# SCZwangxiao/video-ReTaKe

Hardware: NVIDIA B200
Metric: 2048-frame DPSelect+PivotKV frames/s (higher is better)
Workload: dtype bf16

## Files before the change

### video-retake_b200/csrc/pivot_misc.cu

```cuda
#include <climits>

#include <stdlib.h>

#include "rtk_common.cuh"

namespace rtk {

struct RopeParams {
    int heads, L, D, n_pos, forward;
    long long stride_h, stride_l, out_stride_h, out_stride_l;
    int heads2;
    const __nv_bfloat16* x2;
    __nv_bfloat16* out2;
    long long stride_h2, stride_l2, out_stride_h2, out_stride_l2;
    int bound[6];
    float inv_scale2;
};

static bool mrope_bounds(int n_pos, const int32_t* sec, int64_t D, int bound[6]) {
    int acc = 0;
    for (int i = 0; i < 6; ++i) {
        acc += n_pos == 3 ? sec[i % 3] : 0;
        bound[i] = acc;
    }
    return n_pos != 3 || acc == D;
}

__device__ __forceinline__ int rope_pos_row(const RopeParams& p, int c) {
    if (p.n_pos == 1) return 0;
    int i = 0;
    while (i < 5 && c >= p.bound[i]) ++i;
    return i % 3;
}

__global__ void __launch_bounds__(256)
pivot_rope_table_kernel(const long long* __restrict__ pos, const float* __restrict__ inv_freq, RopeParams p, float scaling,
                        __nv_bfloat16* __restrict__ cos_t, __nv_bfloat16* __restrict__ sin_t) {
    pdl_enter();
    const int half = p.D >> 1;
    const long long total = (long long)p.L * p.D;
    for (long long i = (long long)blockIdx.x * blockDim.x + threadIdx.x; i < total; i += (long long)gridDim.x * blockDim.x) {
        const int c = (int)(i % p.D);
        const int l = (int)(i / p.D);
        const long long pv = pos[(size_t)rope_pos_row(p, c) * p.L + l];
        const float ang = inv_freq[c < half ? c : c - half] * (float)pv;
        cos_t[i] = __float2bfloat16_rn(cosf(ang) * scaling);
        sin_t[i] = __float2bfloat16_rn(sinf(ang) * scaling);
    }
}

__device__ __forceinline__ void rope_rotate_pair(float xa, float xb, float cosa, float sina, float cosb, float sinb, int forward,
                                                 float inv_scale2, __nv_bfloat16& oa, __nv_bfloat16& ob) {
    const float ta = round_bf16(xa * cosa), ra = round_bf16(-xb * sina);
    const float tb = round_bf16(xb * cosb), rb = round_bf16(xa * sinb);
    float ya, yb;
    if (forward) {
        ya = ta + ra;
        yb = tb + rb;
    } else {
        ya = round_bf16(ta - ra) * inv_scale2;
        yb = round_bf16(tb - rb) * inv_scale2;
    }
    oa = __float2bfloat16_rn(ya);
    ob = __float2bfloat16_rn(yb);
}

__device__ __forceinline__ void rope_table_entry(const RopeParams& p, const float* __restrict__ inv_freq, const long long* pv,
                                                 int c, float scaling, float& co, float& si) {
    const int half = p.D >> 1;
    const float ang = inv_freq[c < half ? c : c - half] * (float)pv[rope_pos_row(p, c)];
    co = __bfloat162float(__float2bfloat16_rn(cosf(ang) * scaling));
    si = __bfloat162float(__float2bfloat16_rn(sinf(ang) * scaling));
}

#ifndef RTK_UNROPE_TOK
#define RTK_UNROPE_TOK 2
#endif
constexpr int kUnropeTok = RTK_UNROPE_TOK;

__device__ __forceinline__ uint32_t sub_bf16x2_rn(uint32_t a, uint32_t b) {
    uint32_t d;
    asm("sub.rn.bf16x2 %0, %1, %2;" : "=r"(d) : "r"(a), "r"(b));
    return d;
// ... 154 lines not shown
#pragma unroll
            for (int e = 0; e < 8; ++e) {
                const int ca = c0 + e, cb = c0 + e + half;
                const size_t ia = ((size_t)rope_pos_row(p, ca) * p.L + l) * p.D + ca;
                const size_t ib = ((size_t)rope_pos_row(p, cb) * p.L + l) * p.D + cb;
                cav[e] = cos_t[ia]; sav[e] = sin_t[ia]; cbv[e] = cos_t[ib]; sbv[e] = sin_t[ib];
            }
        }
#pragma unroll
        for (int e = 0; e < 8; ++e)
            rope_rotate_pair(__bfloat162float(xl[e]), __bfloat162float(xh[e]), __bfloat162float(cav[e]), __bfloat162float(sav[e]),
                             __bfloat162float(cbv[e]), __bfloat162float(sbv[e]), p.forward, p.inv_scale2, ol[e], oh[e]);
        *reinterpret_cast<uint4*>(dst + c0) = ol4;
        *reinterpret_cast<uint4*>(dst + c0 + half) = oh4;
    }
}

bool key_elision_enabled();

struct KeyElide {
    const uint8_t* keymask[kMaxBatchLayers];
    int32_t* slot[kMaxBatchLayers];
    const __nv_bfloat16* k[kMaxBatchLayers];
    long long k_stride_h[kMaxBatchLayers], k_stride_l[kMaxBatchLayers];
    __nv_bfloat16* kc[kMaxBatchLayers];
    int32_t* n_keys;
    int L, KVH, D;
};

__global__ void __launch_bounds__(1024)
pivot_keymask_scan_kernel(const __grid_constant__ KeyElide e) {
    pdl_enter();
    __shared__ int wsum[32];
    const int layer = blockIdx.x, tid = threadIdx.x, lane = tid & 31, warp = tid >> 5;
    const uint8_t* __restrict__ m = e.keymask[layer];
    int32_t* __restrict__ slot = e.slot[layer];
    const int per = (e.L + 1023) / 1024;
    const int beg = min(tid * per, e.L), end = min(beg + per, e.L);
    int cnt = 0;
    for (int i = beg; i < end; ++i) cnt += !(m && m[i]);
    int inc = cnt;
#pragma unroll
    for (int o = 1; o < 32; o <<= 1) {
        const int n = __shfl_up_sync(0xffffffffu, inc, o);
        if (lane >= o) inc += n;
    }
    if (lane == 31) wsum[warp] = inc;
    __syncthreads();
    if (warp == 0) {
        const int w = wsum[lane];
        int winc = w;
#pragma unroll
        for (int o = 1; o < 32; o <<= 1) {
            const int n = __shfl_up_sync(0xffffffffu, winc, o);
            if (lane >= o) winc += n;
        }
        wsum[lane] = winc - w;
        if (lane == 31) e.n_keys[layer] = winc;
    }
    __syncthreads();
    int base = wsum[warp] + inc - cnt;
    for (int i = beg; i < end; ++i) slot[i] = (m && m[i]) ? -1 : base++;
}

__global__ void __launch_bounds__(256)
pivot_keys_compact_kernel(const __grid_constant__ KeyElide e) {
    pdl_enter();
    const int layer = blockIdx.y;
    const int vpr = e.D >> 3;
    const long long total = (long long)e.L * e.KVH * vpr;
    const int32_t* __restrict__ slot = e.slot[layer];
    for (long long i = (long long)blockIdx.x * blockDim.x + threadIdx.x; i < total; i += (long long)gridDim.x * blockDim.x) {
        const int v = (int)(i % vpr);
        const long long lh = i / vpr;
        const int h = (int)(lh % e.KVH);
        const int l = (int)(lh / e.KVH);
        const int sl = slot[l];
        if (sl < 0) continue;
        const uint4 w = __ldg(reinterpret_cast<const uint4*>(e.k[layer] + h * e.k_stride_h[layer] + l * e.k_stride_l[layer] + v * 8));
        *reinterpret_cast<uint4*>(e.kc[layer] + ((size_t)sl * e.KVH + h) * e.D + v * 8) = w;
    }
}

static int key_elide_prepare(KeyElide& ke, int n, ScoreBatch& sb, cudaStream_t st) {
    RTK_LAUNCH_PDL(pivot_keymask_scan_kernel, (unsigned)n, 1024, 0, st, ke);
    const long long total = (long long)ke.L * ke.KVH * (ke.D >> 3);
    long long gx = (total + 255) / 256;
    if (gx > 148 * 8) gx = 148 * 8;
    RTK_LAUNCH_PDL(pivot_keys_compact_kernel, dim3((unsigned)gx, (unsigned)n), 256, 0, st, ke);
    for (int i = 0; i < n; ++i) {
        sb.kc[i] = ke.kc[i];
        sb.slot[i] = ke.slot[i];
    }
    sb.n_keys = ke.n_keys;
    return 0;
}

static size_t key_elide_bytes(int64_t KVH, int64_t L, int64_t D) {
    return (((size_t)KVH * L * D * 2 + 255) & ~(size_t)255) + (((size_t)L * 4 + 255) & ~(size_t)255);
}

constexpr int kSelThreads = 1024;

__device__ void block_select_top(const uint32_t* keys, int L, int keep, int32_t* out_idx, int* sh ,
                                 int low_bit ) {
    const int tid = threadIdx.x, lane = tid & 31, warp = tid >> 5;
    const int per = (L + kSelThreads - 1) / kSelThreads;
    const int beg = min(tid * per, L), end = min(beg + per, L);
    uint32_t prefix = 0;
    for (int bit = 31; bit >= low_bit; --bit) {
        const uint32_t cand = prefix | (1u << bit);
        int cnt = 0;
        for (int i = beg; i < end; ++i) cnt += (keys[i] >= cand);
        cnt = __reduce_add_sync(0xffffffffu, cnt);
        int* buf = sh + 40 + 32 * (bit & 1);
        if (lane == 0) buf[warp] = cnt;
        __syncthreads();
        const int total = __reduce_add_sync(0xffffffffu, buf[lane]);
        if (total >= keep) prefix = cand;
    }
    __syncthreads();
    if (low_bit > 0 && (!(prefix & 0x80000000u) || (prefix >> low_bit) == (0xffffffffu >> low_bit)))
        prefix |= (1u << low_bit) - 1u;
    int gt = 0, eq = 0;
    for (int i = beg; i < end; ++i) { gt += (keys[i] > prefix); eq += (keys[i] == prefix); }
    auto block_excl_scan = [&](int v, int& total) {
        int inc = v;
#pragma unroll
        for (int o = 1; o < 32; o <<= 1) {
            const int n = __shfl_up_sync(0xffffffffu, inc, o);
            if (lane >= o) inc += n;
        }
        __syncthreads();
        if (lane == 31) sh[1 + warp] = inc;
        __syncthreads();
        if (warp == 0) {
            int w = sh[1 + lane], winc = w;
#pragma unroll
            for (int o = 1; o < 32; o <<= 1) {
                const int n = __shfl_up_sync(0xffffffffu, winc, o);
                if (lane >= o) winc += n;
            }
            sh[1 + lane] = winc - w;
            if (lane == 31) sh[33] = winc;
        }
        __syncthreads();
        total = sh[33];
        return sh[1 + warp] + inc - v;
    };
    int gt_total, eq_total;
    const int gt_before = block_excl_scan(gt, gt_total);
    const int eq_before = block_excl_scan(eq, eq_total);
    const int need = keep - gt_total;
    const int eq_taken_before = min(eq_before, need);
    int slot = gt_before + eq_taken_before;
    int eq_seen = eq_before;
    for (int i = beg; i < end; ++i) {
        const uint32_t k = keys[i];
        bool take = k > prefix;
        if (k == prefix) { take = eq_seen < need; ++eq_seen; }
        if (take) out_idx[slot++] = i;
    }
}

__device__ __forceinline__ void pivot_select_body(const __nv_bfloat16* __restrict__ head_scores, int KVH, int L,
                                                  const uint8_t* __restrict__ keymask, int keep, int32_t* __restrict__ keep_idx,
                                                  __nv_bfloat16* __restrict__ score_out, const long long* __restrict__ tpos,
                                                  long long* __restrict__ tmin_out) {
    extern __shared__ __align__(128) uint8_t smem[];
    uint32_t* keys = reinterpret_cast<uint32_t*>(smem);
    int* sh = reinterpret_cast<int*>(smem + (size_t)L * 4);
    const float rcp = 1.0f / (float)KVH;
// ... 388 lines not shown
    RTK_LAUNCH_PDL(pivot_rope_table_kernel, (unsigned)grid, 256, 0, (cudaStream_t)stream,  (const long long*)pos, inv_freq, p, attention_scaling, (__nv_bfloat16*)cos_out, (__nv_bfloat16*)sin_out);
    return 0;
}

static size_t align256(size_t x) { return (x + 255) & ~(size_t)255; }

extern "C" size_t rtk_pivot_update_batch_workspace_bytes(int64_t H, int64_t KVH, int64_t L, int64_t D, int64_t n_layers) {
    if (H < 1 || KVH < 1 || L < 1 || D < 1 || n_layers < 1) return 0;
    const size_t n = (size_t)(n_layers < kMaxBatchLayers ? n_layers : kMaxBatchLayers);
    return align256(rtk_pivot_score_workspace_bytes(H * (int64_t)n, L)) +
           n * (align256((size_t)H * L * D * 2) + align256((size_t)KVH * L * D * 2)) + align256(n * sizeof(long long)) + 256 +
           n * key_elide_bytes(KVH, L, D) + 256;
}

extern "C" size_t rtk_pivot_update_workspace_bytes(int64_t H, int64_t KVH, int64_t L, int64_t D) {
    return rtk_pivot_update_batch_workspace_bytes(H, KVH, L, D, 1);
}

#ifndef RTK_UNROT_TOKEN_MAJOR
#define RTK_UNROT_TOKEN_MAJOR 1
#endif

static int pivot_update_group(const rtk_pivot_update_args* a, int n, char* ws, cudaStream_t st) {
    const rtk_pivot_update_args& a0 = a[0];
    const int64_t H = a0.H, KVH = a0.KVH, L = a0.L, D = a0.D;
    const bool reforge = a0.reforge != 0;
    const int64_t uq_sh = RTK_UNROT_TOKEN_MAJOR ? D : L * D, uq_sl = RTK_UNROT_TOKEN_MAJOR ? H * D : D;
    const int64_t uk_sh = RTK_UNROT_TOKEN_MAJOR ? D : L * D, uk_sl = RTK_UNROT_TOKEN_MAJOR ? KVH * D : D;
    void* score_ws = ws;                ws += align256(rtk_pivot_score_workspace_bytes(H * n, L));
    char* qu0 = ws;                     ws += (size_t)n * align256((size_t)H * L * D * 2);
    char* ku0 = ws;                     ws += (size_t)n * align256((size_t)KVH * L * D * 2);
    long long* tmin = (long long*)ws;   ws += align256((size_t)n * sizeof(long long)) + 256;
    char* kc0 = ws;                     ws += (size_t)n * align256((size_t)KVH * L * D * 2);
    char* slot0 = ws;                   ws += (size_t)n * align256((size_t)L * 4);
    int32_t* nkeys_ws = (int32_t*)ws;

    BatchLayers t = {};
    ScoreBatch sb = {};
    sb.n = n; sb.H = H; sb.KVH = KVH; sb.L = L; sb.D = D;
    for (int i = 0; i < kMaxBatchLayers; ++i) {
        const rtk_pivot_update_args& x = a[i < n ? i : 0];
        char* qu = qu0 + (size_t)(i < n ? i : 0) * align256((size_t)H * L * D * 2);
        char* ku = ku0 + (size_t)(i < n ? i : 0) * align256((size_t)KVH * L * D * 2);
        t.q[i] = (const __nv_bfloat16*)x.q;       t.q_stride_h[i] = x.q_stride_h;     t.q_stride_l[i] = x.q_stride_l;
        t.k_in[i] = (const __nv_bfloat16*)x.k;    t.kin_stride_h[i] = x.k_stride_h;   t.kin_stride_l[i] = x.k_stride_l;
        t.qu[i] = (__nv_bfloat16*)qu;             t.ku[i] = (__nv_bfloat16*)ku;
        t.k[i] = reforge ? (const __nv_bfloat16*)ku : (const __nv_bfloat16*)x.k;
        t.k_stride_h[i] = reforge ? uk_sh : x.k_stride_h;
        t.k_stride_l[i] = reforge ? uk_sl : x.k_stride_l;
        t.v[i] = (const __nv_bfloat16*)x.v;       t.v_stride_h[i] = x.v_stride_h;     t.v_stride_l[i] = x.v_stride_l;
        t.pos[i] = (const long long*)x.pos;       t.keymask[i] = x.keymask;
        t.k_out[i] = (__nv_bfloat16*)x.k_out;     t.v_out[i] = (__nv_bfloat16*)x.v_out;
        t.out_stride_h[i] = x.out_stride_h;
        t.pos_out[i] = (long long*)x.pos_out;     t.pos_out_stride[i] = x.pos_out_stride > 0 ? x.pos_out_stride : x.keep;
        t.keep_idx[i] = x.keep_idx;               t.head_scores[i] = (const __nv_bfloat16*)x.head_scores;
        if (i < n) {
            sb.q[i] = reforge ? (const void*)qu : x.q;
            sb.k[i] = reforge ? (const void*)ku : x.k;
            sb.q_stride_h[i] = reforge ? uq_sh : x.q_stride_h;   sb.q_stride_l[i] = reforge ? uq_sl : x.q_stride_l;
            sb.k_stride_h[i] = reforge ? uk_sh : x.k_stride_h;   sb.k_stride_l[i] = reforge ? uk_sl : x.k_stride_l;
            sb.head_scores[i] = x.head_scores;
        }
    }
    RopeParams rp = {};
    rp.heads = (int)H; rp.L = (int)L; rp.D = (int)D; rp.n_pos = a0.n_pos; rp.forward = 0;
    rp.out_stride_h = uq_sh; rp.out_stride_l = uq_sl;
    rp.heads2 = (int)KVH; rp.out_stride_h2 = uk_sh; rp.out_stride_l2 = uk_sl;
    rp.inv_scale2 = a0.inv_scale2;
    mrope_bounds(a0.n_pos, a0.mrope_section, D, rp.bound);
    const bool xchg = a0.xchg_world > 1;
    const int64_t score_rows = a0.score_rows > 0 ? a0.score_rows : KVH;
    if (reforge && !a0.skip_score) {
        if (a0.inv_freq) {
            RTK_LAUNCH_PDL(pivot_unrope_qk_batch_kernel, dim3((unsigned)((L + kUnropeTok - 1) / kUnropeTok), (unsigned)n), 256, 0, st, t, a0.inv_freq,
                           a0.attention_scaling, rp);
        } else {
            rp.stride_h = a0.q_stride_h; rp.stride_l = a0.q_stride_l;
            rp.x2 = t.k_in[0]; rp.out2 = t.ku[0]; rp.stride_h2 = a0.k_stride_h; rp.stride_l2 = a0.k_stride_l;
            const int rc = rope_launch(a0.q, a0.cos, a0.sin, t.qu[0], rp, st);
            if (rc) return rc;
        }
    }
    if (!a0.skip_score) {
        bool any_mask = false;
        for (int i = 0; i < n; ++i) any_mask = any_mask || a[i].keymask != nullptr;
        if (any_mask && key_elision_enabled()) {
            KeyElide ke = {};
            ke.L = (int)L; ke.KVH = (int)KVH; ke.D = (int)D; ke.n_keys = nkeys_ws;
            for (int i = 0; i < kMaxBatchLayers; ++i) {
                const int j = i < n ? i : 0;
                ke.keymask[i] = a[j].keymask;
                ke.slot[i] = (int32_t*)(slot0 + (size_t)j * align256((size_t)L * 4));
                ke.k[i] = t.k[j]; ke.k_stride_h[i] = t.k_stride_h[j]; ke.k_stride_l[i] = t.k_stride_l[j];
                ke.kc[i] = (__nv_bfloat16*)(kc0 + (size_t)j * align256((size_t)KVH * L * D * 2));
            }
            int rc = key_elide_prepare(ke, n, sb, st);
            if (rc) return rc;
        }
        if (a0.ev_score_begin) cudaEventRecord((cudaEvent_t)a0.ev_score_begin, st);
        int rc = pivot_score_batch(sb, score_ws, rtk_pivot_score_workspace_bytes(H * n, L), st);
        if (rc) return rc;
        if (a0.ev_score_end) cudaEventRecord((cudaEvent_t)a0.ev_score_end, st);
    }
    if (a0.skip_select) {
        if (xchg) {
            XchgPutBatch xp = {};
            xp.n = (long long)KVH * L; xp.world = a0.xchg_world; xp.rank = a0.xchg_rank;
            for (int i = 0; i < n; ++i) {
                xp.src[i] = (const __nv_bfloat16*)a[i].head_scores;
                for (int r = 0; r < a0.xchg_world; ++r)
                    xp.dst[i][r] = (__nv_bfloat16*)a[i].xchg_scores[r] + (size_t)a0.xchg_rank * KVH * L;
            }
            RTK_LAUNCH_PDL(pivot_xchg_put_batch_kernel, (unsigned)n, 1024, 0, st, xp);
            XchgFlags xf = {};
            xf.world = a0.xchg_world; xf.rank = a0.xchg_rank; xf.epoch = a0.xchg_epoch;
            for (int r = 0; r < a0.xchg_world; ++r) xf.flags[r] = a0.xchg_flags[r];
            RTK_LAUNCH_PDL(pivot_xchg_flag_kernel, 1, 32, 0, st, xf);
        }
        return 0;
    }
    {
        const size_t smem = (size_t)L * 4 + 112 * 4;
        cudaError_t e = cudaFuncSetAttribute(pivot_select_batch_kernel, cudaFuncAttributeMaxDynamicSharedMemorySize, (int)smem);
        if (e != cudaSuccess) return (int)e;
        RTK_LAUNCH_PDL(pivot_select_batch_kernel, (unsigned)n, kSelThreads, smem, st, t, (int)score_rows, (int)L, (int)a0.keep,
                       reforge ? 1 : 0, tmin, (const uint32_t*)(xchg ? a0.xchg_flags[a0.xchg_rank] : nullptr),
                       xchg ? a0.xchg_world : 0, a0.xchg_epoch, xchg_timeout_ns());
    }
    {
        CompactParams p = {};
        p.KVH = (int)KVH; p.L = (int)L; p.D = (int)D; p.keep = (int)a0.keep; p.n_pos = a0.pos ? a0.n_pos : 0; p.reforge = a0.reforge;
        p.ratio = (float)((double)a0.keep / (double)L);
        RopeParams rq = {};
        rq.D = (int)D; rq.n_pos = a0.n_pos; rq.L = (int)a0.keep;
        for (int i = 0; i < 6; ++i) rq.bound[i] = rp.bound[i];
        RTK_LAUNCH_PDL(pivot_compact_rope_batch_kernel, dim3((unsigned)a0.keep, (unsigned)n), 128, 0, st, t, (const long long*)tmin,
                       a0.inv_freq, a0.attention_scaling, p, rq, (reforge && a0.inv_freq) ? 1 : 0);
    }
    return 0;
}

static int update_check(const rtk_pivot_update_args* layers, int64_t n, const void* workspace, size_t workspace_bytes) {
    if (!layers || n < 1 || !workspace) return RTK_E_BADARG;
    const rtk_pivot_update_args& a0 = layers[0];
    const bool scores = !a0.skip_score, selects = !a0.skip_select, xchg = a0.xchg_world > 1;
    if (!scores && !selects) return RTK_E_BADARG;
    if (a0.H < 1 || a0.KVH < 1 || a0.L < 1 || (selects && (a0.keep < 1 || a0.keep > a0.L))) return RTK_E_BADARG;
    if (a0.L > 16384 || a0.D % 16 != 0 || a0.D > 256) return RTK_E_UNSUPPORTED;
    if (scores && ((a0.D != 64 && a0.D != 128) || a0.H % a0.KVH != 0 || a0.H > 256)) return RTK_E_UNSUPPORTED;
    if (xchg) {
        if (n > kMaxBatchLayers) return RTK_E_UNSUPPORTED;
        if (a0.xchg_world > 8 || a0.xchg_rank < 0 || a0.xchg_rank >= a0.xchg_world || (scores && selects)) return RTK_E_BADARG;
    }
    if (a0.reforge && !a0.inv_freq && n > 1) return RTK_E_UNSUPPORTED;
    int bound[6];
    if (a0.reforge && (scores || a0.inv_freq) && !mrope_bounds(a0.n_pos, a0.mrope_section, a0.D, bound)) return RTK_E_UNSUPPORTED;
    if (((uintptr_t)workspace & 255u) != 0) return RTK_E_ALIGN;
    if (workspace_bytes < rtk_pivot_update_batch_workspace_bytes(a0.H, a0.KVH, a0.L, a0.D, n)) return RTK_E_WORKSPACE;
    for (int64_t i = 0; i < n; ++i) {
        const rtk_pivot_update_args& x = layers[i];
        if (!x.q || !x.k || !x.v || !x.k_out || !x.v_out || !x.keep_idx || !x.head_scores) return RTK_E_BADARG;
        if (x.H != a0.H || x.KVH != a0.KVH || x.L != a0.L || x.D != a0.D || x.keep != a0.keep || x.reforge != a0.reforge ||
            x.n_pos != a0.n_pos || x.inv_freq != a0.inv_freq || x.attention_scaling != a0.attention_scaling ||
            x.inv_scale2 != a0.inv_scale2 || x.skip_select != a0.skip_select || x.skip_score != a0.skip_score ||
            x.score_rows != a0.score_rows || x.xchg_world != a0.xchg_world || x.xchg_rank != a0.xchg_rank ||
            x.xchg_epoch != a0.xchg_epoch || (x.pos == nullptr) != (a0.pos == nullptr))
            return RTK_E_UNSUPPORTED;
        for (int j = 0; j < 3; ++j)
            if (x.mrope_section[j] != a0.mrope_section[j]) return RTK_E_UNSUPPORTED;
        if (x.reforge && (!x.pos || !x.pos_out || (!x.inv_freq && (!x.cos || !x.sin)))) return RTK_E_BADARG;
        if (xchg) {
            for (int r = 0; r < a0.xchg_world; ++r)
                if (!x.xchg_scores[r] || !a0.xchg_flags[r]) return RTK_E_BADARG;
            const char* own = (const char*)x.xchg_scores[a0.xchg_rank];
            if (a0.skip_score && (const char*)x.head_scores != own) return RTK_E_BADARG;
            if (a0.skip_select && (const char*)x.head_scores != own + (size_t)a0.xchg_rank * a0.KVH * a0.L * 2) return RTK_E_BADARG;
        }
        if (x.pos && (selects || x.reforge) && (!x.pos_out || x.n_pos < 1 || x.n_pos > 3)) return RTK_E_BADARG;
        uintptr_t ptrs = 0;
        int64_t strides = 0;
        if (scores) {
            ptrs |= (uintptr_t)x.q;
            strides |= x.q_stride_h | x.q_stride_l;
// ... 66 lines not shown
```

### video-retake_b200/csrc/pivot_score.cu

```cuda
#include <cuda.h>

#include "rtk_common.cuh"

namespace rtk {

constexpr int kTile = 128;
constexpr int kHeadDim = 128;
constexpr int kPair = 2;
constexpr int kStages = 2;
constexpr int kASlots = 2;
constexpr int kAccBufs = 4;
constexpr int kStatSlots = kStages + kAccBufs;
constexpr uint32_t kTileBytes = kTile * kHeadDim * 2;
constexpr uint32_t kHalfBytes = kTile * 64 * 2;

struct ScoreSmem {
    static constexpr uint32_t a_tile = 0;
    static constexpr uint32_t b_ring = kASlots * kPair * kTileBytes;
    static constexpr uint32_t stats = b_ring + kStages * kTileBytes;
    static constexpr uint32_t merge = stats + kStatSlots * kTile * 4;
    static constexpr uint32_t bars = merge + 4 * kTile * 2 * 4;
    static constexpr uint32_t n_bars = 4 + 2 * kStages + 2 * kAccBufs + kStatSlots;
    static constexpr uint32_t tmem_ptr = bars + n_bars * 8;
    static constexpr uint32_t total = tmem_ptr + 16;
};

__device__ __forceinline__ void tmem_alloc(uint32_t smem_dst, uint32_t ncols) {
    asm volatile("tcgen05.alloc.cta_group::1.sync.aligned.shared::cta.b32 [%0], %1;" ::"r"(smem_dst), "r"(ncols) : "memory");
    asm volatile("tcgen05.relinquish_alloc_permit.cta_group::1.sync.aligned;" ::: "memory");
}
__device__ __forceinline__ void tmem_dealloc(uint32_t taddr, uint32_t ncols) {
    asm volatile("tcgen05.dealloc.cta_group::1.sync.aligned.b32 %0, %1;" ::"r"(taddr), "r"(ncols) : "memory");
}
__device__ __forceinline__ void tc_fence_before() { asm volatile("tcgen05.fence::before_thread_sync;" ::: "memory"); }
__device__ __forceinline__ void tc_fence_after() { asm volatile("tcgen05.fence::after_thread_sync;" ::: "memory"); }
__device__ __forceinline__ void tc_commit(uint32_t bar) {
    asm volatile("tcgen05.commit.cta_group::1.mbarrier::arrive::one.shared::cluster.b64 [%0];" ::"r"(bar) : "memory");
}
__device__ __forceinline__ void umma_bf16(uint32_t tmem_d, uint64_t adesc, uint64_t bdesc, uint32_t idesc, uint32_t accum) {
    asm volatile(
        "{\n\t.reg .pred p;\n\t"
        "setp.ne.b32 p, %4, 0;\n\t"
        "tcgen05.mma.cta_group::1.kind::f16 [%0], %1, %2, %3, p;\n\t}"
        ::"r"(tmem_d), "l"(adesc), "l"(bdesc), "r"(idesc), "r"(accum)
        : "memory");
}
__device__ __forceinline__ void tmem_ld_wait() { asm volatile("tcgen05.wait::ld.sync.aligned;" ::: "memory"); }
__device__ __forceinline__ void tmem_ld64(uint32_t taddr, uint32_t (&r)[64]) {
    asm volatile(
        "tcgen05.ld.sync.aligned.32x32b.x64.b32 "
        "{%0, %1, %2, %3, %4, %5, %6, %7, %8, %9, %10, %11, %12, %13, %14, %15, "
        "%16, %17, %18, %19, %20, %21, %22, %23, %24, %25, %26, %27, %28, %29, %30, %31, "
        "%32, %33, %34, %35, %36, %37, %38, %39, %40, %41, %42, %43, %44, %45, %46, %47, "
        "%48, %49, %50, %51, %52, %53, %54, %55, %56, %57, %58, %59, %60, %61, %62, %63}, [%64];"
        : "=r"(r[0]), "=r"(r[1]), "=r"(r[2]), "=r"(r[3]), "=r"(r[4]), "=r"(r[5]), "=r"(r[6]), "=r"(r[7]),
          "=r"(r[8]), "=r"(r[9]), "=r"(r[10]), "=r"(r[11]), "=r"(r[12]), "=r"(r[13]), "=r"(r[14]), "=r"(r[15]),
          "=r"(r[16]), "=r"(r[17]), "=r"(r[18]), "=r"(r[19]), "=r"(r[20]), "=r"(r[21]), "=r"(r[22]), "=r"(r[23]),
          "=r"(r[24]), "=r"(r[25]), "=r"(r[26]), "=r"(r[27]), "=r"(r[28]), "=r"(r[29]), "=r"(r[30]), "=r"(r[31]),
          "=r"(r[32]), "=r"(r[33]), "=r"(r[34]), "=r"(r[35]), "=r"(r[36]), "=r"(r[37]), "=r"(r[38]), "=r"(r[39]),
          "=r"(r[40]), "=r"(r[41]), "=r"(r[42]), "=r"(r[43]), "=r"(r[44]), "=r"(r[45]), "=r"(r[46]), "=r"(r[47]),
          "=r"(r[48]), "=r"(r[49]), "=r"(r[50]), "=r"(r[51]), "=r"(r[52]), "=r"(r[53]), "=r"(r[54]), "=r"(r[55]),
          "=r"(r[56]), "=r"(r[57]), "=r"(r[58]), "=r"(r[59]), "=r"(r[60]), "=r"(r[61]), "=r"(r[62]), "=r"(r[63])
        : "r"(taddr)
        : "memory");
}
__device__ __forceinline__ void add_bf16_pair(float& acc_lo, float& acc_hi, uint32_t packed) {
    asm("{\n\t.reg .b16 lo, hi;\n\t"
        "mov.b32 {lo, hi}, %2;\n\t"
        "add.rn.f32.bf16 %0, lo, %0;\n\t"
        "add.rn.f32.bf16 %1, hi, %1;\n\t}"
        : "+f"(acc_lo), "+f"(acc_hi)
        : "r"(packed));
}

__device__ __forceinline__ void tma_load_3d(uint32_t dst, const CUtensorMap* map, int c0, int c1, int c2, uint32_t bar) {
    asm volatile(
        "cp.async.bulk.tensor.3d.shared::cluster.global.tile.mbarrier::complete_tx::bytes [%0], [%1, {%3, %4, %5}], [%2];"
        ::"r"(dst), "l"(reinterpret_cast<uint64_t>(map)), "r"(bar), "r"(c0), "r"(c1), "r"(c2)
        : "memory");
}
__device__ __forceinline__ float ex2f(float x) {
    float y;
    asm("ex2.approx.ftz.f32 %0, %1;" : "=f"(y) : "f"(x));
// ... 376 lines not shown
    if (p0.x > -INFINITY) lt += p0.y * ex2f((p0.x - mn) * kLog2e);
    if (p1.x > -INFINITY) lt += p1.y * ex2f((p1.x - mn) * kLog2e);
    if (p2.x > -INFINITY) lt += p2.y * ex2f((p2.x - mn) * kLog2e);
    stats[o] = (q < L) ? fmaf(mn, kLog2e, lg2f(lt)) : INFINITY;
}

struct HeadScoreOut {
    __nv_bfloat16* p[kMaxBatchLayers];
    const int32_t* slot[kMaxBatchLayers];
    int KVH;
};

__global__ void pivot_head_reduce_kernel(const float* __restrict__ colsum_part, int H, int G, int L, int Lpad,
                                         const __grid_constant__ HeadScoreOut out) {
    pdl_enter();
    const int k = blockIdx.x * blockDim.x + threadIdx.x;
    const int g = blockIdx.y;
    if (k >= L) return;
    const size_t hl = (size_t)H * Lpad;
    const int layer = g / out.KVH;
    int col = k;
    if (out.slot[layer]) {
        col = out.slot[layer][k];
        if (col < 0) {
            out.p[layer][(size_t)(g - layer * out.KVH) * L + k] = __float2bfloat16_rn(1.0f);
            return;
        }
    }
    float v[4] = {0.f, 0.f, 0.f, 0.f};
    for (int j = 0; j < G; ++j) {
        const size_t o = (size_t)(g * G + j) * Lpad + col;
        v[j & 3] += round_bf16((colsum_part[o] + colsum_part[hl + o]) + colsum_part[2 * hl + o]);
    }
    const float s = ((v[0] + v[1]) + v[2]) + v[3];
    out.p[layer][(size_t)(g - layer * out.KVH) * L + k] = __float2bfloat16_rn(s * (1.0f / (float)G));
}

typedef CUresult (*EncodeTiledFn)(CUtensorMap*, CUtensorMapDataType, cuuint32_t, void*, const cuuint64_t*, const cuuint64_t*,
                                  const cuuint32_t*, const cuuint32_t*, CUtensorMapInterleave, CUtensorMapSwizzle,
                                  CUtensorMapL2promotion, CUtensorMapFloatOOBfill);

static EncodeTiledFn get_encode_fn() {
    static EncodeTiledFn fn = nullptr;
    if (fn) return fn;
    void* p = nullptr;
    cudaDriverEntryPointQueryResult qres;
    if (cudaGetDriverEntryPoint("cuTensorMapEncodeTiled", &p, cudaEnableDefault, &qres) != cudaSuccess ||
        qres != cudaDriverEntryPointSuccess)
        return nullptr;
    fn = reinterpret_cast<EncodeTiledFn>(p);
    return fn;
}

static int make_map(CUtensorMap* map, const void* ptr, int64_t heads, int64_t L, int64_t D, int64_t stride_h,
                    int64_t stride_l, int* dim1_is_l) {
    EncodeTiledFn enc = get_encode_fn();
    if (!enc) return RTK_E_DRIVER;
    const bool l_first = (heads == 1) || (stride_l <= stride_h);
    *dim1_is_l = l_first ? 1 : 0;
    cuuint64_t dims[3] = {(cuuint64_t)D, (cuuint64_t)(l_first ? L : heads), (cuuint64_t)(l_first ? heads : L)};
    cuuint64_t strides[2] = {(cuuint64_t)((l_first ? stride_l : stride_h) * 2), (cuuint64_t)((l_first ? stride_h : stride_l) * 2)};
    if (heads == 1) strides[1] = (cuuint64_t)(stride_l * 2) * (cuuint64_t)L;
    cuuint32_t box[3] = {64u, (cuuint32_t)(l_first ? kTile : 1), (cuuint32_t)(l_first ? 1 : kTile)};
    cuuint32_t estr[3] = {1u, 1u, 1u};
    CUresult r = enc(map, CU_TENSOR_MAP_DATA_TYPE_BFLOAT16, 3, const_cast<void*>(ptr), dims, strides, box, estr,
                     CU_TENSOR_MAP_INTERLEAVE_NONE, CU_TENSOR_MAP_SWIZZLE_128B, CU_TENSOR_MAP_L2_PROMOTION_L2_256B,
                     CU_TENSOR_MAP_FLOAT_OOB_FILL_NONE);
    return r == CUDA_SUCCESS ? 0 : RTK_E_DRIVER;
}

}

using namespace rtk;

extern "C" size_t rtk_pivot_score_workspace_bytes(int64_t H, int64_t L) {
    if (H < 1 || L < 1) return 0;
    const size_t lpad = (size_t)((L + kTile - 1) / kTile) * kTile;
    return 10 * (size_t)H * lpad * sizeof(float);
}

namespace rtk {

template <int NL>
static int score_launch(const ScoreBatch& b, ScoreParams prm, cudaStream_t st) {
    ScoreMaps<NL> maps;
    for (int l = 0; l < b.n; ++l) {
        int ql = 0, kl = 0;
        int rc = make_map(&maps.q[l], b.q[l], b.H, b.L, b.D, b.q_stride_h[l], b.q_stride_l[l], &ql);
        if (rc) return rc;
        rc = make_map(&maps.k[l], b.k[l], b.KVH, b.L, b.D, b.k_stride_h[l], b.k_stride_l[l], &kl);
        if (rc) return rc;
        if (l == 0) { prm.q_dim1_is_l = ql; prm.k_dim1_is_l = kl; }
        else if (ql != prm.q_dim1_is_l || kl != prm.k_dim1_is_l) return RTK_E_UNSUPPORTED;
        if (prm.n_keys) {
            int cl = 0;
            rc = make_map(&maps.kc[l], b.kc[l], b.KVH, b.L, b.D, b.D, b.KVH * b.D, &cl);
            if (rc) return rc;
            prm.kc_dim1_is_l = cl;
        } else {
            maps.kc[l] = maps.k[l];
        }
    }
    for (int l = b.n; l < NL; ++l) { maps.q[l] = maps.q[0]; maps.k[l] = maps.k[0]; maps.kc[l] = maps.kc[0]; }
    int dev = 0, sms = 0;
    cudaGetDevice(&dev);
    cudaDeviceGetAttribute(&sms, cudaDevAttrMultiProcessorCount, dev);
    const int units = prm.Hl * ((prm.nt + kPair - 1) / kPair);
    const long long gmax = (long long)units * prm.nt / ((prm.nt + 1) / 2);
    const int grid = (int)(gmax < sms ? (gmax < 1 ? 1 : gmax) : sms);
    const size_t smem = ScoreSmem::total + 1024;
    cudaError_t e = cudaFuncSetAttribute(pivot_score_kernel<1, NL>, cudaFuncAttributeMaxDynamicSharedMemorySize, (int)smem);
    if (e != cudaSuccess) return (int)e;
    e = cudaFuncSetAttribute(pivot_score_kernel<2, NL>, cudaFuncAttributeMaxDynamicSharedMemorySize, (int)smem);
    if (e != cudaSuccess) return (int)e;
    HeadScoreOut out;
    out.KVH = (int)b.KVH;
    for (int l = 0; l < kMaxBatchLayers; ++l) {
        out.p[l] = reinterpret_cast<__nv_bfloat16*>(b.head_scores[l < b.n ? l : 0]);
        out.slot[l] = prm.n_keys ? b.slot[l < b.n ? l : 0] : nullptr;
    }
    RTK_LAUNCH_PDL((pivot_score_kernel<1, NL>), grid, kScoreThreads2, smem, st, maps, prm);
    dim3 g1((unsigned)((prm.nt * kTile + 255) / 256), (unsigned)prm.H);
    RTK_LAUNCH_PDL(pivot_stats_merge_kernel, g1, 256, 0, st, prm.ml_part, prm.H, prm.L, prm.nt * kTile, prm.stats);
    RTK_LAUNCH_PDL((pivot_score_kernel<2, NL>), grid, kScoreThreads2, smem, st, maps, prm);
    dim3 g2((unsigned)((prm.L + 255) / 256), (unsigned)(b.KVH * b.n));
    RTK_LAUNCH_PDL(pivot_head_reduce_kernel, g2, 256, 0, st, prm.colsum_part, prm.H, prm.G, prm.L, prm.nt * kTile, out);
    return 0;
}

int pivot_score_batch(const ScoreBatch& b, void* workspace, size_t workspace_bytes, cudaStream_t st) {
    if (b.n < 1 || b.n > kMaxBatchLayers || !workspace || b.H < 1 || b.KVH < 1 || b.L < 1) return RTK_E_BADARG;
    if ((b.D != 64 && b.D != 128) || b.H % b.KVH != 0 || b.L > 16384 || b.H > 256) return RTK_E_UNSUPPORTED;
    if (((uintptr_t)workspace & 15u) != 0) return RTK_E_ALIGN;
    for (int l = 0; l < b.n; ++l) {
        if (!b.q[l] || !b.k[l] || !b.head_scores[l]) return RTK_E_BADARG;
        if ((((uintptr_t)b.q[l] | (uintptr_t)b.k[l]) & 15u) != 0) return RTK_E_ALIGN;
        if ((b.q_stride_h[l] | b.q_stride_l[l] | b.k_stride_h[l] | b.k_stride_l[l]) % 8 != 0) return RTK_E_ALIGN;
    }
    if (workspace_bytes < rtk_pivot_score_workspace_bytes(b.H * b.n, b.L)) return RTK_E_WORKSPACE;

    ScoreParams prm;
    prm.H = (int)(b.H * b.n);
    prm.Hl = (int)b.H;
    prm.G = (int)(b.H / b.KVH);
    prm.L = (int)b.L;
    prm.nt = (int)((b.L + kTile - 1) / kTile);
    prm.n_atoms = (int)(b.D / 64);
    prm.q_dim1_is_l = prm.k_dim1_is_l = prm.kc_dim1_is_l = 0;
    prm.n_keys = b.n_keys;
    if (b.n_keys)
        for (int l = 0; l < b.n; ++l)
            if (!b.kc[l] || !b.slot[l] || ((uintptr_t)b.kc[l] & 15u) != 0) return RTK_E_BADARG;
    const float sq = (float)sqrt((double)b.D);
    prm.inv_sqrt_d = 1.0f / sq;
    const size_t plane = (size_t)prm.H * prm.nt * kTile;
    prm.ml_part = reinterpret_cast<float2*>(workspace);
    prm.stats = reinterpret_cast<float*>(workspace) + 6 * plane;
    prm.colsum_part = prm.stats + plane;
    return b.n == 1 ? score_launch<1>(b, prm, st) : score_launch<kMaxBatchLayers>(b, prm, st);
}

}

extern "C" int rtk_pivot_score(const void* q, int64_t H, int64_t q_stride_h, int64_t q_stride_l, const void* k, int64_t KVH,
                               int64_t k_stride_h, int64_t k_stride_l, int64_t L, int64_t D, void* head_scores,
                               void* workspace, size_t workspace_bytes, void* stream) {
    RTK_NVTX("rtk_pivot_score");
    if (!q || !k || !head_scores || !workspace || H < 1 || KVH < 1 || L < 1) return RTK_E_BADARG;
    ScoreBatch b = {};
    b.n = 1; b.H = H; b.KVH = KVH; b.L = L; b.D = D;
    b.q[0] = q; b.k[0] = k; b.head_scores[0] = head_scores;
    b.q_stride_h[0] = q_stride_h; b.q_stride_l[0] = q_stride_l; b.k_stride_h[0] = k_stride_h; b.k_stride_l[0] = k_stride_l;
    return pivot_score_batch(b, workspace, workspace_bytes, (cudaStream_t)stream);
}
```

### video-retake_b200/csrc/rtk_common.cuh

```cuda
#pragma once

#include <cuda_bf16.h>
#include <cuda_runtime.h>
#include <nvtx3/nvToolsExt.h>
#include <stdint.h>

#include "../../include/rtk_b200.h"

namespace rtk {

extern long long g_launches;

#define RTK_CHECK_LAUNCH()                                   \
    do {                                                     \
        ++::rtk::g_launches;                                 \
        cudaError_t e__ = cudaGetLastError();                \
        if (e__ != cudaSuccess) return (int)e__;             \
    } while (0)

constexpr int kWarp = 32;

struct NvtxRange {
    explicit NvtxRange(const char* name) { nvtxRangePushA(name); }
    ~NvtxRange() { nvtxRangePop(); }
    NvtxRange(const NvtxRange&) = delete;
    NvtxRange& operator=(const NvtxRange&) = delete;
};
#define RTK_NVTX(name) ::rtk::NvtxRange nvtx_range__(name)

struct DisAux {
    float* sim;
    float* nrm;
    long long si, sp;
};
int dpselect_sim_nrm(const void* x, int64_t T, int64_t N, int64_t C, DisAux aux, cudaStream_t st);

constexpr int kMaxBatchLayers = 32;
struct ScoreBatch {
    int n;
    int64_t H, KVH, L, D;
    const void* q[kMaxBatchLayers];
    const void* k[kMaxBatchLayers];
    void* head_scores[kMaxBatchLayers];
    int64_t q_stride_h[kMaxBatchLayers], q_stride_l[kMaxBatchLayers], k_stride_h[kMaxBatchLayers], k_stride_l[kMaxBatchLayers];
    const void* kc[kMaxBatchLayers];
    const int32_t* slot[kMaxBatchLayers];
    const int32_t* n_keys;
};
int pivot_score_batch(const ScoreBatch& b, void* workspace, size_t workspace_bytes, cudaStream_t st);

__device__ __forceinline__ void pdl_trigger() { asm volatile("griddepcontrol.launch_dependents;" ::: "memory"); }
__device__ __forceinline__ void pdl_wait() { asm volatile("griddepcontrol.wait;" ::: "memory"); }
#ifndef RTK_PDL_EARLY_SMALL
#define RTK_PDL_EARLY_SMALL 1
#endif
#ifndef RTK_PDL_EARLY_SCORE
#define RTK_PDL_EARLY_SCORE 1
#endif
__device__ __forceinline__ void pdl_enter() {
    if (RTK_PDL_EARLY_SMALL) pdl_trigger();
    pdl_wait();
}

bool pdl_enabled();

template <typename... KArgs, typename... Args>
static inline cudaError_t launch_pdl(void (*kern)(KArgs...), dim3 grid, dim3 block, size_t smem, cudaStream_t st,
                                     Args&&... args) {
    cudaLaunchConfig_t cfg = {};
    cfg.gridDim = grid;
    cfg.blockDim = block;
    cfg.dynamicSmemBytes = smem;
    cfg.stream = st;
    cudaLaunchAttribute attr[1];
    attr[0].id = cudaLaunchAttributeProgrammaticStreamSerialization;
    attr[0].val.programmaticStreamSerializationAllowed = 1;
    cfg.attrs = attr;
    cfg.numAttrs = pdl_enabled() ? 1 : 0;
    return cudaLaunchKernelEx(&cfg, kern, static_cast<KArgs>(args)...);
}
#define RTK_LAUNCH_PDL(kern, grid, block, smem, st, ...)                                                  \
    do {                                                                                                  \
        ++::rtk::g_launches;                                                                              \
        cudaError_t le__ = ::rtk::launch_pdl(kern, dim3(grid), dim3(block), (size_t)(smem), st, __VA_ARGS__); \
        if (le__ != cudaSuccess) return (int)le__;                                                        \
    } while (0)

__device__ __forceinline__ float bf16lo_to_f32(uint32_t packed) { return __uint_as_float(packed << 16); }
__device__ __forceinline__ float bf16hi_to_f32(uint32_t packed) { return __uint_as_float(packed & 0xffff0000u); }

__device__ __forceinline__ uint32_t pack_bf16x2_rn(float lo, float hi) {
    uint32_t d;
    asm("cvt.rn.bf16x2.f32 %0, %1, %2;" : "=r"(d) : "f"(hi), "f"(lo));
    return d;
}
__device__ __forceinline__ float round_bf16(float x) {
    return __bfloat162float(__float2bfloat16_rn(x));
}
__device__ __forceinline__ uint32_t mul_bf16x2_rn(uint32_t a, uint32_t b) {
    uint32_t d;
    asm("mul.rn.bf16x2 %0, %1, %2;" : "=r"(d) : "r"(a), "r"(b));
    return d;
}

__device__ __forceinline__ void fma_sq_bf16x2(float& acc_lo, float& acc_hi, uint32_t p) {
    asm("{\n\t.reg .b16 lo, hi;\n\t"
        "mov.b32 {lo, hi}, %2;\n\t"
        "fma.rn.f32.bf16 %0, lo, lo, %0;\n\t"
        "fma.rn.f32.bf16 %1, hi, hi, %1;\n\t}"
        : "+f"(acc_lo), "+f"(acc_hi)
        : "r"(p));
}
__device__ __forceinline__ void add_bf16x2(float& acc_lo, float& acc_hi, uint32_t p) {
    asm("{\n\t.reg .b16 lo, hi;\n\t"
        "mov.b32 {lo, hi}, %2;\n\t"
        "add.rn.f32.bf16 %0, lo, %0;\n\t"
        "add.rn.f32.bf16 %1, hi, %1;\n\t}"
        : "+f"(acc_lo), "+f"(acc_hi)
        : "r"(p));
}
__device__ __forceinline__ uint32_t scale_bf16x2_rn(uint32_t p, float s) {
    return pack_bf16x2_rn(bf16lo_to_f32(p) * s, bf16hi_to_f32(p) * s);
}

__device__ __forceinline__ uint32_t f32_to_ordered(float v) {
    uint32_t x = __float_as_uint(v);
    uint32_t mask = (x & 0x80000000u) ? 0xffffffffu : 0x80000000u;
    return (v == v) ? (x ^ mask) : 0xffffffffu;
}

__device__ __forceinline__ uint32_t smem_u32(const void* p) { return (uint32_t)__cvta_generic_to_shared(p); }

__device__ __forceinline__ void mbar_init(uint32_t bar, uint32_t count) {
    asm volatile("mbarrier.init.shared::cta.b64 [%0], %1;" ::"r"(bar), "r"(count) : "memory");
}
__device__ __forceinline__ void fence_mbar_init() {
    asm volatile("fence.mbarrier_init.release.cluster;" ::: "memory");
}
__device__ __forceinline__ void fence_proxy_async() {
    asm volatile("fence.proxy.async.shared::cta;" ::: "memory");
}
__device__ __forceinline__ void mbar_arrive_expect_tx(uint32_t bar, uint32_t bytes) {
    asm volatile("mbarrier.arrive.expect_tx.shared::cta.b64 _, [%0], %1;" ::"r"(bar), "r"(bytes) : "memory");
}
__device__ __forceinline__ void mbar_arrive(uint32_t bar) {
    asm volatile("mbarrier.arrive.shared::cta.b64 _, [%0];" ::"r"(bar) : "memory");
}
__device__ __forceinline__ bool mbar_try_wait(uint32_t bar, uint32_t parity) {
    uint32_t ok;
    asm volatile(
        "{\n\t.reg .pred p;\n\t"
        "mbarrier.try_wait.parity.shared::cta.b64 p, [%1], %2;\n\t"
        "selp.u32 %0, 1, 0, p;\n\t}"
        : "=r"(ok)
        : "r"(bar), "r"(parity)
        : "memory");
    return ok != 0;
}
__device__ __forceinline__ void mbar_wait(uint32_t bar, uint32_t parity) {
    while (!mbar_try_wait(bar, parity)) {
    }
}
__device__ __forceinline__ void bulk_g2s(uint32_t dst_smem, const void* src, uint32_t bytes, uint32_t bar) {
    asm volatile("cp.async.bulk.shared::cluster.global.mbarrier::complete_tx::bytes [%0], [%1], %2, [%3];" ::"r"(dst_smem),
                 "l"(src), "r"(bytes), "r"(bar)
                 : "memory");
}
// ... 26 lines not shown
```

Baseline: 3605.

## Overlap key-compaction gather with score pass 1 on a side stream

Moves the masked-key compaction kernel onto a per-stream side stream, sized to fit in the SM resources left beside the score kernel, so it can run concurrently with the first scoring pass. The main stream waits on an event before the stats-merge kernel, which is the first consumer of compacted keys. This aims to hide the gather's memory traffic behind the score kernel, at the cost of losing PDL on that edge, adding event and stream overhead, and possible contention for SM resources. An environment variable can disable the overlap.

```diff
diff --git a/video-retake_b200/csrc/pivot_misc.cu b/video-retake_b200/csrc/pivot_misc.cu
--- a/video-retake_b200/csrc/pivot_misc.cu
+++ b/video-retake_b200/csrc/pivot_misc.cu
@@ -1,4 +1,7 @@
 #include <climits>
+#include <map>
+#include <mutex>
+#include <utility>
 
 #include <stdlib.h>
 
@@ -319,12 +322,73 @@
     }
 }
 
-static int key_elide_prepare(KeyElide& ke, int n, ScoreBatch& sb, cudaStream_t st) {
+struct SideStream {
+    cudaStream_t s = nullptr;
+    cudaEvent_t fork = nullptr, keys = nullptr;
+    int sms = 0, gather_ctas = 0;
+};
+constexpr int kGatherThreads = 128;
+
+static int side_stream(cudaStream_t st, SideStream** out) {
+    static std::mutex mu;
+    static std::map<std::pair<int, cudaStream_t>, SideStream> streams;
+    int dev = 0;
+    cudaError_t e = cudaGetDevice(&dev);
+    if (e != cudaSuccess) return (int)e;
+    std::lock_guard<std::mutex> lock(mu);
+    SideStream& ss = streams[{dev, st}];
+    if (!ss.s) {
+        cudaStream_t s = nullptr;
+        e = cudaStreamCreateWithFlags(&s, cudaStreamNonBlocking);
+        if (e == cudaSuccess) e = cudaEventCreateWithFlags(&ss.fork, cudaEventDisableTiming);
+        if (e == cudaSuccess) e = cudaEventCreateWithFlags(&ss.keys, cudaEventDisableTiming);
+        if (e == cudaSuccess)
+            e = cudaFuncSetAttribute(pivot_keys_compact_kernel, cudaFuncAttributePreferredSharedMemoryCarveout,
+                                     cudaSharedmemCarveoutMaxShared);
+        if (e == cudaSuccess) e = cudaDeviceGetAttribute(&ss.sms, cudaDevAttrMultiProcessorCount, dev);
+        if (e != cudaSuccess) {
+            streams.erase({dev, st});
+            return (int)e;
+        }
+        ss.gather_ctas = ctas_next_to_score((const void*)pivot_keys_compact_kernel, kGatherThreads, 0);
+        ss.s = s;
+    }
+    *out = &ss;
+    return 0;
+}
+
+static bool key_gather_overlap_enabled() {
+    static const bool on = [] {
+        const char* e = getenv("RTK_NO_KEY_GATHER_OVERLAP");
+        return !(e && e[0] && e[0] != '0');
+    }();
+    return on;
+}
+
+static int key_elide_prepare(KeyElide& ke, int n, ScoreBatch& sb, cudaStream_t st, cudaEvent_t* keys_ready) {
+    *keys_ready = nullptr;
+    SideStream* side = nullptr;
+    if (key_gather_overlap_enabled()) {
+        const int rc = side_stream(st, &side);
+        if (rc) return rc;
+        if (side->gather_ctas < 1) side = nullptr;
+    }
     RTK_LAUNCH_PDL(pivot_keymask_scan_kernel, (unsigned)n, 1024, 0, st, ke);
-    const long long total = (long long)ke.L * ke.KVH * (ke.D >> 3);
-    long long gx = (total + 255) / 256;
-    if (gx > 148 * 8) gx = 148 * 8;
-    RTK_LAUNCH_PDL(pivot_keys_compact_kernel, dim3((unsigned)gx, (unsigned)n), 256, 0, st, ke);
+    if (side) {
+        cudaError_t e = cudaEventRecord(side->fork, st);
+        if (e == cudaSuccess) e = cudaStreamWaitEvent(side->s, side->fork, 0);
+        if (e != cudaSuccess) return (int)e;
+        const int gx = side->sms * side->gather_ctas / n;
+        RTK_LAUNCH(pivot_keys_compact_kernel, dim3((unsigned)(gx > 0 ? gx : 1), (unsigned)n), kGatherThreads, 0, side->s, ke);
+        e = cudaEventRecord(side->keys, side->s);
+        if (e != cudaSuccess) return (int)e;
+        *keys_ready = side->keys;
+    } else {
+        const long long total = (long long)ke.L * ke.KVH * (ke.D >> 3);
+        long long gx = (total + 255) / 256;
+        if (gx > 148 * 8) gx = 148 * 8;
+        RTK_LAUNCH_PDL(pivot_keys_compact_kernel, dim3((unsigned)gx, (unsigned)n), 256, 0, st, ke);
+    }
     for (int i = 0; i < n; ++i) {
         sb.kc[i] = ke.kc[i];
         sb.slot[i] = ke.slot[i];
@@ -879,6 +943,7 @@
         }
     }
     if (!a0.skip_score) {
+        cudaEvent_t keys_ready = nullptr;
         bool any_mask = false;
         for (int i = 0; i < n; ++i) any_mask = any_mask || a[i].keymask != nullptr;
         if (any_mask && key_elision_enabled()) {
@@ -891,11 +956,11 @@
                 ke.k[i] = t.k[j]; ke.k_stride_h[i] = t.k_stride_h[j]; ke.k_stride_l[i] = t.k_stride_l[j];
                 ke.kc[i] = (__nv_bfloat16*)(kc0 + (size_t)j * align256((size_t)KVH * L * D * 2));
             }
-            int rc = key_elide_prepare(ke, n, sb, st);
+            int rc = key_elide_prepare(ke, n, sb, st, &keys_ready);
             if (rc) return rc;
         }
         if (a0.ev_score_begin) cudaEventRecord((cudaEvent_t)a0.ev_score_begin, st);
-        int rc = pivot_score_batch(sb, score_ws, rtk_pivot_score_workspace_bytes(H * n, L), st);
+        int rc = pivot_score_batch(sb, score_ws, rtk_pivot_score_workspace_bytes(H * n, L), st, keys_ready);
         if (rc) return rc;
         if (a0.ev_score_end) cudaEventRecord((cudaEvent_t)a0.ev_score_end, st);
     }
diff --git a/video-retake_b200/csrc/pivot_score.cu b/video-retake_b200/csrc/pivot_score.cu
--- a/video-retake_b200/csrc/pivot_score.cu
+++ b/video-retake_b200/csrc/pivot_score.cu
@@ -1,4 +1,6 @@
 #include <cuda.h>
+
+#include <algorithm>
 
 #include "rtk_common.cuh"
 
@@ -541,7 +543,7 @@
 namespace rtk {
 
 template <int NL>
-static int score_launch(const ScoreBatch& b, ScoreParams prm, cudaStream_t st) {
+static int score_launch(const ScoreBatch& b, ScoreParams prm, cudaEvent_t keys_ready, cudaStream_t st) {
     ScoreMaps<NL> maps;
     for (int l = 0; l < b.n; ++l) {
         int ql = 0, kl = 0;
@@ -580,14 +582,20 @@
     }
     RTK_LAUNCH_PDL((pivot_score_kernel<1, NL>), grid, kScoreThreads2, smem, st, maps, prm);
     dim3 g1((unsigned)((prm.nt * kTile + 255) / 256), (unsigned)prm.H);
-    RTK_LAUNCH_PDL(pivot_stats_merge_kernel, g1, 256, 0, st, prm.ml_part, prm.H, prm.L, prm.nt * kTile, prm.stats);
+    if (keys_ready) {
+        const cudaError_t we = cudaStreamWaitEvent(st, keys_ready, 0);
+        if (we != cudaSuccess) return (int)we;
+        RTK_LAUNCH(pivot_stats_merge_kernel, g1, 256, 0, st, prm.ml_part, prm.H, prm.L, prm.nt * kTile, prm.stats);
+    } else {
+        RTK_LAUNCH_PDL(pivot_stats_merge_kernel, g1, 256, 0, st, prm.ml_part, prm.H, prm.L, prm.nt * kTile, prm.stats);
+    }
     RTK_LAUNCH_PDL((pivot_score_kernel<2, NL>), grid, kScoreThreads2, smem, st, maps, prm);
     dim3 g2((unsigned)((prm.L + 255) / 256), (unsigned)(b.KVH * b.n));
     RTK_LAUNCH_PDL(pivot_head_reduce_kernel, g2, 256, 0, st, prm.colsum_part, prm.H, prm.G, prm.L, prm.nt * kTile, out);
     return 0;
 }
 
-int pivot_score_batch(const ScoreBatch& b, void* workspace, size_t workspace_bytes, cudaStream_t st) {
+int pivot_score_batch(const ScoreBatch& b, void* workspace, size_t workspace_bytes, cudaStream_t st, cudaEvent_t keys_ready) {
     if (b.n < 1 || b.n > kMaxBatchLayers || !workspace || b.H < 1 || b.KVH < 1 || b.L < 1) return RTK_E_BADARG;
     if ((b.D != 64 && b.D != 128) || b.H % b.KVH != 0 || b.L > 16384 || b.H > 256) return RTK_E_UNSUPPORTED;
     if (((uintptr_t)workspace & 15u) != 0) return RTK_E_ALIGN;
@@ -616,7 +624,32 @@
     prm.ml_part = reinterpret_cast<float2*>(workspace);
     prm.stats = reinterpret_cast<float*>(workspace) + 6 * plane;
     prm.colsum_part = prm.stats + plane;
-    return b.n == 1 ? score_launch<1>(b, prm, st) : score_launch<kMaxBatchLayers>(b, prm, st);
+    return b.n == 1 ? score_launch<1>(b, prm, keys_ready, st) : score_launch<kMaxBatchLayers>(b, prm, keys_ready, st);
+}
+
+int ctas_next_to_score(const void* kern, int threads, size_t dyn_smem) {
+    cudaFuncAttributes fs, fk;
+    if (cudaFuncGetAttributes(&fs, (const void*)pivot_score_kernel<1, kMaxBatchLayers>) != cudaSuccess ||
+        cudaFuncGetAttributes(&fk, kern) != cudaSuccess)
+        return 0;
+    int dev = 0, regs_sm = 0, smem_sm = 0, thr_sm = 0, blk_sm = 0, reserved = 0, alone = 0;
+    cudaGetDevice(&dev);
+    cudaDeviceGetAttribute(&regs_sm, cudaDevAttrMaxRegistersPerMultiprocessor, dev);
+    cudaDeviceGetAttribute(&smem_sm, cudaDevAttrMaxSharedMemoryPerMultiprocessor, dev);
+    cudaDeviceGetAttribute(&thr_sm, cudaDevAttrMaxThreadsPerMultiProcessor, dev);
+    cudaDeviceGetAttribute(&blk_sm, cudaDevAttrMaxBlocksPerMultiprocessor, dev);
+    cudaDeviceGetAttribute(&reserved, cudaDevAttrReservedSharedMemoryPerBlock, dev);
+    if (cudaOccupancyMaxActiveBlocksPerMultiprocessor(&alone, kern, threads, dyn_smem) != cudaSuccess) return 0;
+    auto regs = [](int per_thread, int thr) { return ((per_thread * 32 + 255) / 256 * 256) * ((thr + 31) / 32); };
+    const long long left_regs = regs_sm - regs(fs.numRegs, kScoreThreads2);
+    const long long left_smem = smem_sm - (long long)(fs.sharedSizeBytes + ScoreSmem::total + 1024 + reserved);
+    const long long left_thr = thr_sm - kScoreThreads2;
+    long long n = blk_sm - 1;
+    n = std::min(n, left_regs / regs(fk.numRegs, threads));
+    n = std::min(n, left_smem / (long long)(fk.sharedSizeBytes + dyn_smem + reserved));
+    n = std::min(n, left_thr / threads);
+    n = std::min(n, (long long)alone);
+    return n > 0 ? (int)n : 0;
 }
 
 }
diff --git a/video-retake_b200/csrc/rtk_common.cuh b/video-retake_b200/csrc/rtk_common.cuh
--- a/video-retake_b200/csrc/rtk_common.cuh
+++ b/video-retake_b200/csrc/rtk_common.cuh
@@ -47,7 +47,9 @@
     const int32_t* slot[kMaxBatchLayers];
     const int32_t* n_keys;
 };
-int pivot_score_batch(const ScoreBatch& b, void* workspace, size_t workspace_bytes, cudaStream_t st);
+int pivot_score_batch(const ScoreBatch& b, void* workspace, size_t workspace_bytes, cudaStream_t st,
+                      cudaEvent_t keys_ready = nullptr);
+int ctas_next_to_score(const void* kern, int threads, size_t dyn_smem);
 
 __device__ __forceinline__ void pdl_trigger() { asm volatile("griddepcontrol.launch_dependents;" ::: "memory"); }
 __device__ __forceinline__ void pdl_wait() { asm volatile("griddepcontrol.wait;" ::: "memory"); }
@@ -65,8 +67,8 @@
 bool pdl_enabled();
 
 template <typename... KArgs, typename... Args>
-static inline cudaError_t launch_pdl(void (*kern)(KArgs...), dim3 grid, dim3 block, size_t smem, cudaStream_t st,
-                                     Args&&... args) {
+static inline cudaError_t launch_kernel(bool pdl, void (*kern)(KArgs...), dim3 grid, dim3 block, size_t smem, cudaStream_t st,
+                                        Args&&... args) {
     cudaLaunchConfig_t cfg = {};
     cfg.gridDim = grid;
     cfg.blockDim = block;
@@ -76,13 +78,24 @@
     attr[0].id = cudaLaunchAttributeProgrammaticStreamSerialization;
     attr[0].val.programmaticStreamSerializationAllowed = 1;
     cfg.attrs = attr;
-    cfg.numAttrs = pdl_enabled() ? 1 : 0;
+    cfg.numAttrs = pdl ? 1 : 0;
     return cudaLaunchKernelEx(&cfg, kern, static_cast<KArgs>(args)...);
+}
+template <typename... KArgs, typename... Args>
+static inline cudaError_t launch_pdl(void (*kern)(KArgs...), dim3 grid, dim3 block, size_t smem, cudaStream_t st,
+                                     Args&&... args) {
+    return launch_kernel(pdl_enabled(), kern, grid, block, smem, st, static_cast<Args&&>(args)...);
 }
 #define RTK_LAUNCH_PDL(kern, grid, block, smem, st, ...)                                                  \
     do {                                                                                                  \
         ++::rtk::g_launches;                                                                              \
         cudaError_t le__ = ::rtk::launch_pdl(kern, dim3(grid), dim3(block), (size_t)(smem), st, __VA_ARGS__); \
+        if (le__ != cudaSuccess) return (int)le__;                                                        \
+    } while (0)
+#define RTK_LAUNCH(kern, grid, block, smem, st, ...)                                                      \
+    do {                                                                                                  \
+        ++::rtk::g_launches;                                                                              \
+        cudaError_t le__ = ::rtk::launch_kernel(false, kern, dim3(grid), dim3(block), (size_t)(smem), st, __VA_ARGS__); \
         if (le__ != cudaSuccess) return (int)le__;                                                        \
     } while (0)
 
```

Result: no change. 3613, median of 6 (+0.2%).
